# afermg/aliby

Hardware: AMD Instinct MI355X
Metric: FOV tiles/sec (whole node) (higher is better)
Workload: dtype u16 pixels, f64 feature accumulators, f32 dynamics, bfloat16 U-Net

## Files before the change

### aliby_amd/_lib.py

```python

from __future__ import annotations

import ctypes as C
import os
import threading
from pathlib import Path

import numpy as np

_HERE = Path(__file__).resolve().parent
LIB_PATH = Path(os.environ["ALIBY_HIP_LIB"]) if os.environ.get("ALIBY_HIP_LIB") else _HERE / "libaliby_hip.so"

OK, ERR_INVALID, ERR_OVERFLOW, ERR_HIP, ERR_TOO_LARGE, ERR_UNSUPPORTED = range(6)
U16, F32 = 0, 1
U8W = 4
U64, F64 = 2, 3
RED_MAX, RED_ADD, RED_DIV = 0, 1, 2


class AlibyHipError(RuntimeError):
    pass


class aliby_object(C.Structure):
    _fields_ = [
        ("tile", C.c_int32),
        ("label", C.c_int32),
        ("y0", C.c_int32),
        ("x0", C.c_int32),
        ("y1", C.c_int32),
        ("x1", C.c_int32),
        ("area", C.c_int32),
        ("pad_", C.c_int32),
    ]


class aliby_pq_column(C.Structure):
    _fields_ = [("name", C.c_char_p), ("type", C.c_int32), ("reserved", C.c_int32)]


class aliby_npy_member(C.Structure):
    _fields_ = [("name", C.c_char_p), ("descr", C.c_char_p), ("shape", C.POINTER(C.c_int64)), ("data", C.c_void_p),
                ("ndim", C.c_int32), ("itemsize", C.c_int32)]


PQ_F64, PQ_I64, PQ_U16, PQ_STR = range(4)

OBJECT_DTYPE = np.dtype(
    [("tile", "<i4"), ("label", "<i4"), ("y0", "<i4"), ("x0", "<i4"), ("y1", "<i4"), ("x1", "<i4"),
     ("area", "<i4"), ("pad_", "<i4")]
)

_vp, _i, _sz = C.c_void_p, C.c_int, C.c_size_t
_ip = C.POINTER(C.c_int32)

_SIGNATURES = {
    "aliby_abi_version": (_i, []),
    "aliby_last_error": (C.c_char_p, []),
    "aliby_ctx_create": (_i, [_i, C.POINTER(_vp)]),
    "aliby_ctx_destroy": (_i, [_vp]),
    "aliby_device_info": (_i, [_vp, C.POINTER(_i), C.POINTER(_i), C.POINTER(_sz), C.c_char_p, _i]),
    "aliby_malloc": (_i, [_vp, _sz, C.POINTER(_vp)]),
    "aliby_free": (_i, [_vp, _vp]),
    "aliby_memcpy_h2d": (_i, [_vp, _vp, _vp, _sz, _vp]),
    "aliby_memcpy_d2h": (_i, [_vp, _vp, _vp, _sz, _vp]),
    "aliby_memset": (_i, [_vp, _vp, _i, _sz, _vp]),
    "aliby_stream_sync": (_i, [_vp, _vp]),
    "aliby_crop_pad_u16": (_i, [_vp, _vp, _i, _i, _i, _i, _vp, _i, _i, _i, _vp, _vp, _vp]),
    "aliby_reduce_z": (_i, [_vp, _vp, _i, _sz, _i, _sz, _i, _vp, _i, _vp]),
    "aliby_label_max": (_i, [_vp, _vp, _i, _i, _i, _vp, _vp]),
    "aliby_object_table": (_i, [_vp, _vp, _i, _i, _i, _vp, _vp, _vp, _vp]),
    "aliby_relabel_sequential": (_i, [_vp, _vp, _i, _i, _i, _vp, _vp]),
    "aliby_select_project_u16": (_i, [_vp, _vp, _i, _i, _i, _i, _i, _i, _vp, _vp]),
    "aliby_normalize99_u16": (_i, [_vp, _vp, _i, _i, _i, C.c_double, C.c_double, _vp, _vp, _vp]),
    "aliby_make_tiles": (_i, [_vp, _vp, _i, _i, _i, _i, _i, _i, _i, _i, _i, _i, _i, _vp, _vp, _i, _vp, _vp]),
    "aliby_average_tiles": (_i, [_vp, _vp, _i, _i, _i, _i, _i, _i, _i, _i, _i, _i, _i, _vp, _vp, _vp, _vp, _vp, _vp]),
    "aliby_nn_fused_act_bf16": (_i, [_vp, _vp, _vp, _vp, _vp, _vp, _vp, _vp, _i, _i, _i, _i, _i, _i, _i, _i, _vp]),
    "aliby_nn_conv3x3_bf16": (_i, [_vp, _vp, _vp, _vp, _vp, _vp, _i, _vp, _vp, _i, _i, _i, _i, _i, _i, _i, _i, _i, _i, _i, _vp, _vp]),
    "aliby_nn_conv3x3_deep_bf16": (_i, [_vp, _vp, _vp, _vp, _vp, _vp, _i, _vp, _vp, _i, _i, _i, _i, _i, _i, _i, _vp]),
    "aliby_nn_conv3x3_deep16_bf16": (_i, [_vp, _vp, _vp, _vp, _vp, _vp, _i, _vp, _vp, _i, _i, _i, _i, _i, _i, _i, _vp]),
    "aliby_nn_pack_conv3x3_deep16_bf16": (_i, [_vp, _vp, _i, _i, _vp, _vp]),
    "aliby_nn_maxpool2_bf16": (_i, [_vp, _vp, _vp, _i, _i, _i, _i, _vp]),
    "aliby_debug_conv_deep_trace": (_i, [_vp, _vp]),
    "aliby_track_stitch": (_i, [_vp, _vp, _vp, _i, _i, _i, _vp, _vp, _vp, _vp, _vp, _vp, C.c_double, _vp, _vp, _vp]),
    "aliby_debug_conv_trace": (_i, [_vp, _vp]),
    "aliby_features_coloc_pairs": (_i, [_vp, _vp, _vp, _i, _i, _i, _i, _i, _vp, _i, _vp, _i, _i, _vp, _i, C.c_double, C.c_double, _vp, _vp, _vp]),
    "aliby_trap_gauss1d": (_i, [_vp, _vp, _vp, _i, _i, _i, _vp, _i, _i, _vp]),
    "aliby_trap_warp": (_i, [_vp, _vp, _i, _i, _vp, _i, _i, _vp, _i, C.c_double, _vp]),
    "aliby_trap_entropy": (_i, [_vp, _vp, _i, _i, _i, _vp, _vp]),
    "aliby_trap_morph": (_i, [_vp, _vp, _vp, _i, _i, _i, _i, _i, _vp]),
    "aliby_trap_label": (_i, [_vp, _vp, _i, _i, _vp, _vp]),
    "aliby_trap_region_sums": (_i, [_vp, _vp, _i, _i, _vp, _vp]),
    "aliby_trap_match_template": (_i, [_vp, _vp, _i, _i, _vp, _i, _i, _vp, _i, _i, C.c_double, C.c_double, _vp]),
    "aliby_trap_maxfilter1d": (_i, [_vp, _vp, _vp, _i, _i, _i, _i, _vp]),
    "aliby_tiff_probe": (_i, [C.c_char_p, _vp, C.c_char_p, _i]),
    "aliby_ingest_tiff_planes": (_i, [_vp, _vp, _vp, _i, _i, _i, _i, _vp, _sz, _i, _i, _vp]),
    "aliby_ingest_inflate": (_i, [_i, _vp, _sz, _vp, _sz, _vp]),
    "aliby_nn_pack_conv3x3_bf16": (_i, [_vp, _vp, _i, _i, _i, _vp, _vp]),
    "aliby_nn_pack_conv1x1_bf16": (_i, [_vp, _vp, _i, _i, _i, _vp, _vp]),
    "aliby_nn_conv3x3_proj_bf16": (_i, [_vp, _vp, _vp, _vp, _vp, _vp, _i, _vp, _i, _i, _i, _i, _i, _vp, _vp, _i, _vp]),
    "aliby_nn_conv3x3_head_bf16": (_i, [_vp, _vp, _vp, _vp, _vp, _vp, _i, _vp, _vp, _i, _i, _i, _i, _i, _i, _vp, _vp, _vp, _vp, _i, _vp, _vp]),
    "aliby_nn_conv3x3_pair_bf16": (_i, [_vp, _vp, _vp, _vp, _vp, _vp, _vp, _i, _vp, _vp, _vp, _i, _vp, _vp, _i, _i, _i, _vp, _vp, _vp, _vp, _vp,
                                        _i, _vp, _vp]),
    "aliby_nn_first_pair_bf16": (_i, [_vp, _vp, _i, _i, _i, _i, _vp, _vp, _vp, _vp, _vp, _vp, _vp, _vp, _vp, _vp]),
    "aliby_nn_conv1x1_bf16": (_i, [_vp, _vp, _vp, _vp, _vp, _i, _i, _i, _i, _i, _vp]),
    "aliby_nn_first_conv_bf16": (_i, [_vp, _vp, _i, _i, _i, _i, _vp, _vp, _vp, _vp, _vp, _vp]),
    "aliby_nn_style_bf16": (_i, [_vp, _vp, _i, _i, _i, _i, _vp, _vp, _i, _vp, _vp, _vp]),
    "aliby_nn_out_head_bf16": (_i, [_vp, _vp, _vp, _vp, _vp, _vp, _i, _i, _i, _i, _i, _vp, _vp]),
    "aliby_nn_nhwc_to_nchw_f32": (_i, [_vp, _vp, _i, _i, _i, _i, _i, _vp, _vp, _vp]),
    "aliby_nn_tiles_to_nhwc8_bf16": (_i, [_vp, _vp, _i, _i, _i, _i, _vp, _vp, _vp, _vp, _vp]),
    "aliby_masks_workspace_bytes": (_sz, [_i, _i, _i]),
    "aliby_masks_from_flows": (_i, [_vp, _vp, _vp, _i, _i, _i, _i, C.c_float, C.c_float, _i, C.c_float, _vp, _sz,
                                    _vp, _vp, _vp, _vp]),
    "aliby_features_intensity": (_i, [_vp, _vp, _vp, _i, _i, _i, _i, _i, _i, _vp, _i, _i, _i, _vp, _i, _i, _vp]),
    "aliby_features_sizeshape": (_i, [_vp, _vp, _i, _i, _i, _vp, _i, _i, _i, _i, _vp, _i, _i, _vp]),
    "aliby_features_feret": (_i, [_vp, _vp, _i, _i, _i, _vp, _i, _i, _vp, _i, _i, _vp]),
    "aliby_object_mec": (_i, [_vp, _vp, _i, _i, _i, _vp, _i, _i, _vp, _vp]),
    "aliby_features_zernike": (_i, [_vp, _vp, _vp, _i, _i, _i, _i, _i, _i, _vp, _i, _vp, _i, _vp, _i, _i, _vp]),
    "aliby_features_radial_zernikes_multi": (_i, [_vp, _vp, _vp, _i, _i, _i, _i, _i, _vp, _vp, _i, _vp, _i, _vp, _vp, _i, _vp]),
    "aliby_features_texture": (_i, [_vp, _vp, _vp, _i, _i, _i, _i, _i, _i, _vp, _i, _i, _i, _i, _i, _i, _vp, _i, _i, _vp]),
    "aliby_radial_geometry": (_i, [_vp, _vp, _i, _i, _i, _vp, _i, _i, _i, _i, _vp, _vp]),
    "aliby_features_radial_distribution": (_i, [_vp, _vp, _vp, _vp, _i, _i, _i, _i, _i, _i, _vp, _i, _i, _vp, _i, _i, _vp]),
    "aliby_features_cell_ratio": (_i, [_vp, _vp, _vp, _i, _i, _i, _i, _i, _i, _i, _vp, _i, _i, _vp, _vp]),
    "aliby_features_trap_background": (_i, [_vp, _vp, _vp, _i, _i, _i, _i, _i, _i, _vp, _vp]),
    "aliby_granularity_workspace_bytes": (_sz, [_i, _i, _i, _i, C.c_double, C.c_double]),
    "aliby_features_granularity": (_i, [_vp, _vp, _vp, _i, _i, _i, _i, _i, _i, _vp, _i, C.c_double, C.c_double, _i, _i, _i,
                                        _vp, _sz, _vp, _i, _i, _vp]),
    "aliby_radial_geometry_unscaled": (_i, [_vp, _vp, _i, _i, _i, _vp, _i, _i, _i, _i, C.c_double, _vp, _vp]),
    "aliby_features_radial_distribution_rings": (_i, [_vp, _vp, _vp, _vp, _i, _i, _i, _i, _i, _i, _vp, _i, _i, _i, _vp, _i, _i, _vp]),
    "aliby_features_cell": (_i, [_vp, _vp, _vp, _i, _i, _i, _i, _i, _i, _vp, _i, _i, _i, _i, _vp, _i, _i, _vp]),
    "aliby_features_coloc": (_i, [_vp, _vp, _vp, _i, _i, _i, _i, _i, _i, _i, _vp, _i, _i, _vp, _i, _i, _i, _i, _i,
                                  C.c_double, C.c_double, _vp, _vp, _vp]),
    "aliby_labels_apply_lut": (_i, [_vp, _vp, _i, _i, _i, _vp, _vp, _vp, _vp]),
    "aliby_features_intensity3d": (_i, [_vp, _vp, _vp, _i, _i, _i, _i, _i, _i, _vp, _vp, _i, _i, _vp]),
    "aliby_parquet_write": (_i, [C.c_char_p, _vp, _i, _vp, _i, _vp, _vp, _i]),
    "aliby_npz_write": (_i, [C.c_char_p, _vp, _i, _i]),
    "aliby_host_codecs": (_i, [C.POINTER(_i), C.POINTER(_i)]),
    "aliby_host_copy": (_i, [_vp, _vp, _sz, _i]),
    "aliby_object_ranks": (_i, [_vp, _vp, _vp, _i, _i, _i, _i, _i, _i, _vp, _i, _i, _vp, _vp, _vp]),
}

_lib = None


def exported_symbols() -> list[str]:
    return sorted(_SIGNATURES)


def load() -> C.CDLL:
    global _lib
    if _lib is not None:
        return _lib
    if not LIB_PATH.exists():
        raise AlibyHipError(
            f"{LIB_PATH} is missing: build it with `python -c 'import __graft_entry__ as g; g.build()'` "
            "(make -C aliby_amd/csrc). There is no CPU fallback for the HIP path."
        )
    try:
        import torch
    except Exception:
        pass
    lib = C.CDLL(str(LIB_PATH), mode=getattr(os, "RTLD_NOW", 2))
# ... 80 lines not shown
```

### aliby_amd/segment/fused_unet.py

```python

from __future__ import annotations

import os

import torch
import torch.nn.functional as F

from aliby_amd import _lib
from aliby_amd.extraction.engine import _ptr, _stream_ptr

CL = torch.channels_last


def _bn_affine(bn):
    s = bn.weight.float() / torch.sqrt(bn.running_var.float() + bn.eps)
    t = bn.bias.float() - bn.running_mean.float() * s
    return s.contiguous(), t.contiguous()


class _Unit:

    def __init__(self, seq, dtype, pad_in=None):
        bn, conv = seq[0], seq[-1]
        self.scale, self.shift = _bn_affine(bn)
        w = conv.weight.detach().float()
        if pad_in is not None and w.shape[1] < pad_in:
            w = F.pad(w, (0, 0, 0, 0, 0, pad_in - w.shape[1]))
            self.scale = F.pad(self.scale, (0, pad_in - self.scale.shape[0]), value=1.0)
            self.shift = F.pad(self.shift, (0, pad_in - self.shift.shape[0]))
        self.w = w.to(dtype).contiguous(memory_format=CL)
        self.w32 = w.contiguous()
        self.wpk = None
        self.bias = conv.bias.detach().float().contiguous()
        self.pad = conv.padding


class _Proj:

    def __init__(self, seq, dtype, pad_in=None):
        bn, conv = seq[0], seq[-1]
        s, t = _bn_affine(bn)
        w = conv.weight.detach().float()
        b = conv.bias.detach().float() + (w[:, :, 0, 0] @ t)
        w = w * s[None, :, None, None]
        if pad_in is not None and w.shape[1] < pad_in:
            w = F.pad(w, (0, 0, 0, 0, 0, pad_in - w.shape[1]))
        self.w = w.to(dtype).contiguous(memory_format=CL)
        self.w32 = w[:, :, 0, 0].contiguous()
        self.wpk = None
        self.wpk1 = None
        self.bias = b.contiguous()


_MFMA_SHAPES = {(32, 32, False), (32, 64, False), (64, 64, False), (64, 32, True), (64, 64, True), (64, 128, False), (64, 128, True)}
_POOL_SHAPES = {(32, 32, False), (32, 64, False), (64, 64, False), (64, 128, False)}


class FusedUNet:
    @property
    def h(self):
        return self.eng.ctx.handle

    def __init__(self, net, eng, dtype=torch.bfloat16, mfma_levels=(0, 1, 2, 3)):
        assert dtype == torch.bfloat16, "the fused kernels are bf16"
        self.eng, self.dtype = eng, dtype
        self.mfma_levels = tuple(mfma_levels)
        self.fused_head = os.environ.get("ALIBY_NET_FUSED_HEAD", "1") != "0"
        self.fused_pair = os.environ.get("ALIBY_NET_FUSED_PAIR", "1") != "0"
        self.pair_head = os.environ.get("ALIBY_NET_PAIR_HEAD", "0") != "0"
        self.fused_first = os.environ.get("ALIBY_NET_FUSED_FIRST", "1") != "0"
        self.deep_kernel = os.environ.get("ALIBY_CONV_DEEP", "1") != "0"
        self.conv_stats = {}
        self.lib = _lib.load_fast() if os.environ.get("ALIBY_FAST_LAUNCH", "1") != "0" else eng.lib
        net = net.float().eval()
        self.down = []
        for i, blk in enumerate(net.down):
            pad = 8 if i == 0 else None
            d = dict(proj=_Proj(blk.proj, dtype, pad), u=[_Unit(blk.conv[0], dtype, pad)] + [_Unit(blk.conv[k], dtype) for k in (1, 2, 3)])
            d["pb1"] = (d["proj"].bias + d["u"][1].bias).contiguous()
            d["shift1_b0"] = (d["u"][1].scale * d["u"][0].bias + d["u"][1].shift).contiguous()
            self.down.append(d)
        self.up = []
        for blk in net.up:
            d = dict(proj=_Proj(blk.proj, dtype), u=[_Unit(blk.conv0, dtype)])
            for su in (blk.conv1, blk.conv2, blk.conv3):
                u = _Unit(su.conv, dtype)
                u.full_w = su.full.weight.detach().float().t().contiguous()
                u.full_b = su.full.bias.detach().float()
                d["u"].append(u)
            d["pb1"] = (d["proj"].bias + d["u"][1].bias).contiguous()
            self.up.append(d)
        ws, bs, off = [], [], 0
        for d in self.up:
            for k in d["u"][1:]:
                ws.append(k.full_w * k.scale[None, :])
                bs.append(k.full_b * k.scale + k.shift)
                k.style_slice = (off, off + k.scale.numel())
                off += k.scale.numel()
        self.style_w = torch.cat(ws, dim=1).contiguous()
        self.style_b = torch.cat(bs).contiguous()
        self.first_w = net.down[0].conv[0][-1].weight.detach().float().to(dtype).float().contiguous()
        self.out = _Unit(net.output, dtype)
        self.out_w = self.out.w32[:, :, 0, 0].to(dtype).float().contiguous()
        self.cin = net.nbase[0]
        self.bytes_moved = 0

    def _new(self, n, c, h, w):
        return torch.empty((n, c, h, w), dtype=self.dtype, device="cuda", memory_format=CL)

    def _fused(self, A, B=None, want_sum=False, act=None, shift=None, upA=False, upB=False, relu=True, bias=None):
        n, c = A.shape[0], A.shape[1]
        H = A.shape[2] * (2 if upA else 1)
        W = A.shape[3] * (2 if upA else 1)
        S = self._new(n, c, H, W) if want_sum else None
        T = self._new(n, c, H, W) if act is not None else None
        per_sample = 0
        sh = None
        if act is not None:
            sh = shift if shift is not None else act.shift
            per_sample = self._sps(sh)
        timer = self.eng.timed("fused_pointwise")
        if timer.active:
            self.bytes_moved += 2 * (A.numel() + (B.numel() if B is not None else 0) + (n * c * H * W) * ((S is not None) + (T is not None)))
        with timer:
          _lib.check(self.lib.aliby_nn_fused_act_bf16(
            self.h, _ptr(A), _ptr(B) if B is not None else 0, _ptr(S) if S is not None else 0, _ptr(T) if T is not None else 0,
            _ptr(bias) if bias is not None else 0,
            _ptr(act.scale) if act is not None else 0, _ptr(sh) if sh is not None else 0, n, H, W, c, 1 if upA else 0,
            1 if upB else 0, 1 if relu else 0, per_sample, _stream_ptr()))
        return S, T

    @staticmethod
    def _conv(x, unit, pad=1):
        return F.conv2d(x, unit.w, None, padding=pad)

    def _proj(self, x, proj):
        n, cin, H, W = x.shape
        cout = proj.w32.shape[0]
        if cin not in (32, 64, 128, 256) or not (cout in (32, 64) or cout % 128 == 0) or proj.w32.shape[1] != cin:
            return self._conv(x, proj, pad=0)
        if proj.wpk1 is None:
            proj.wpk1 = torch.empty(cout * cin, dtype=torch.bfloat16, device="cuda")
            _lib.check(self.lib.aliby_nn_pack_conv1x1_bf16(self.h, _ptr(proj.w32), cout, cin, cin, _ptr(proj.wpk1), _stream_ptr()))
        out = self._new(n, cout, H, W)
        with self.eng.timed("conv1x1_mfma"):
            _lib.check(self.lib.aliby_nn_conv1x1_bf16(self.h, _ptr(x), _ptr(proj.wpk1), 0, _ptr(out), n, H, W, cin, cout, _stream_ptr()))
        return out

    def _unit(self, x, unit, shift=None, bias=None, res=None, res_up=False, in_up=False, pool=False):
        n, cin, cout = x.shape[0], x.shape[1], unit.w32.shape[0]
        H, W = (x.shape[2] * 2, x.shape[3] * 2) if in_up else (x.shape[2], x.shape[3])
        out = self._new(n, cout, H, W)
        pooled = self._new(n, cout, H // 2, W // 2) if pool else None
        if self.deep_kernel and cout % 128 == 0 and cin in (64, 128, 256) and W <= 56 and (H + 1) * (W + 2) >= 226 + 2 * (W + 2):
            self._launch_deep(x, unit, out, shift, bias, res, res_up, in_up)
            if pool:
                with self.eng.timed("maxpool"):
                    _lib.check(self.lib.aliby_nn_maxpool2_bf16(self.h, _ptr(out), _ptr(pooled), n, H, W, cout, _stream_ptr()))
            return (out, pooled) if pool else out
        if (cin, cout, bool(in_up)) in (_POOL_SHAPES if pool else _MFMA_SHAPES):
            self._launch_unit(x, unit, (0, cin), (0, cout), out, shift, bias, res, res_up, in_up, pooled)
            return (out, pooled) if pool else out
        ns = 128 if cout > 128 else cout
        ks = 64 if cin > 64 else cin
        assert cin % ks == 0 and cout % ns == 0 and (ks, ns, bool(in_up)) in _MFMA_SHAPES, (cin, cout, in_up)
        for n0 in range(0, cout, ns):
            cur, cur_up = res, res_up
            for k0 in range(0, cin, ks):
                last = k0 + ks == cin
                self._launch_unit(x, unit, (k0, k0 + ks), (n0, n0 + ns), out, shift, bias if last else None, cur, cur_up, in_up,
                                  pooled if last else None)
                cur, cur_up = out, False
        return (out, pooled) if pool else out

    def _pack(self, unit):
        cout, cin = unit.w32.shape[0], unit.w32.shape[1]
        if unit.wpk is None:
            unit.wpk = {}
        key = (0, cin, 0, cout)
        if key not in unit.wpk:
            pk = torch.empty(cout * cin * 9, dtype=torch.bfloat16, device="cuda")
            _lib.check(self.lib.aliby_nn_pack_conv3x3_bf16(self.h, _ptr(unit.w32), cout, cin, cin, _ptr(pk), _stream_ptr()))
            unit.wpk[key] = pk
        return unit.wpk[key]

    def _pair(self, x, ua, ub, shift_a, shift_b, bias_a, bias_b, res, pool=False, head_out=None):
        n, cin, H, W = x.shape
        sa = ua.shift if shift_a is None else shift_a
        sb = ub.shift if shift_b is None else shift_b
        out = None if head_out is not None else self._new(n, 32, H, W)
        pooled = self._new(n, 32, H // 2, W // 2) if pool else None
        group = "conv3x3_mfma_pair"
        timer = self.eng.timed(group)
        if timer.active:
            st = self.conv_stats.setdefault(group, [0, 0])
            st[0] += 2 * (x.numel() + res.numel()) + (2 * x.numel() if out is not None else 4 * head_out.numel()) + (x.numel() // 2 if pool else 0)
            st[1] += 2 * 2 * 9 * 32 * 32 * n * H * W
        hd = self.out
        with timer:
            _lib.check(self.lib.aliby_nn_conv3x3_pair_bf16(
                self.h, _ptr(x), _ptr(self._pack(ua)), _ptr(self._pack(ub)), _ptr(out) if out is not None else 0, _ptr(ua.scale), _ptr(sa),
                self._sps(sa), _ptr(bias_a), _ptr(ub.scale), _ptr(sb), self._sps(sb), _ptr(bias_b), _ptr(res), n, H, W,
                _ptr(pooled) if pooled is not None else 0,
                _ptr(hd.scale) if head_out is not None else 0, _ptr(hd.shift) if head_out is not None else 0,
                _ptr(self.out_w) if head_out is not None else 0, _ptr(hd.bias) if head_out is not None else 0,
                self.out_w.shape[0] if head_out is not None else 0, _ptr(head_out) if head_out is not None else 0, _stream_ptr()))
        return (out, pooled) if pool else out

    def _first_pair(self, tiles, d):
        n, cin, H, W = tiles.shape
        u, proj = d["u"], d["proj"]
        wpk1 = self._pack(u[1])
        if proj.wpk is None:
            proj.wpk = torch.empty(32 * 16, dtype=torch.bfloat16, device="cuda")
            _lib.check(self.lib.aliby_nn_pack_conv1x1_bf16(self.h, _ptr(proj.w32), 32, proj.w32.shape[1], 16, _ptr(proj.wpk), _stream_ptr()))
        out = self._new(n, 32, H, W)
        group = "conv3x3_mfma_first_pair"
        timer = self.eng.timed(group)
        if timer.active:
            st = self.conv_stats.setdefault(group, [0, 0])
            st[0] += 4 * tiles.numel() + 2 * out.numel()
            st[1] += 2 * (9 * cin + 9 * 32 + cin) * 32 * n * H * W
        with timer:
            _lib.check(self.lib.aliby_nn_first_pair_bf16(
                self.h, _ptr(tiles), n, cin, H, W, _ptr(u[0].scale), _ptr(u[0].shift), _ptr(self.first_w), _ptr(wpk1), _ptr(u[1].scale),
                _ptr(d["shift1_b0"]), _ptr(d["pb1"]), _ptr(proj.wpk), _ptr(out), _stream_ptr()))
        return out

    def _unit_head(self, x, unit, shift, bias, res, y):
        n, cin, H, W = x.shape
        cout = unit.w32.shape[0]
        if unit.wpk is None:
            unit.wpk = {}
        key = (0, cin, 0, cout)
        if key not in unit.wpk:
            pk = torch.empty(cout * cin * 9, dtype=torch.bfloat16, device="cuda")
            _lib.check(self.lib.aliby_nn_pack_conv3x3_bf16(self.h, _ptr(unit.w32), cout, cin, cin, _ptr(pk), _stream_ptr()))
            unit.wpk[key] = pk
        sh = unit.shift if shift is None else shift
        group = "conv3x3_mfma_head"
        timer = self.eng.timed(group)
        if timer.active:
            st = self.conv_stats.setdefault(group, [0, 0])
            st[0] += 2 * (x.numel() + res.numel()) + 4 * y.numel()
            st[1] += 2 * (9 * cin + y.shape[1]) * cout * n * H * W
        with timer:
            _lib.check(self.lib.aliby_nn_conv3x3_head_bf16(
                self.h, _ptr(x), _ptr(unit.wpk[key]), 0, _ptr(unit.scale), _ptr(sh), self._sps(sh), _ptr(bias), _ptr(res), 0, n, H, W,
                cin, cout, _ptr(self.out.scale), _ptr(self.out.shift), _ptr(self.out_w), _ptr(self.out.bias), self.out_w.shape[0], _ptr(y),
                _stream_ptr()))

    def _unit_proj(self, x, unit, shift, bias, x_in, proj):
        n, cin, H, W = x.shape
        cout = unit.w32.shape[0]
        pc_pad = 16 if cin == 32 else 32
        if unit.wpk is None:
            unit.wpk = {}
        key = (0, cin, 0, cout)
        if key not in unit.wpk:
            pk = torch.empty(cout * cin * 9, dtype=torch.bfloat16, device="cuda")
            _lib.check(self.lib.aliby_nn_pack_conv3x3_bf16(self.h, _ptr(unit.w32), cout, cin, cin, _ptr(pk), _stream_ptr()))
            unit.wpk[key] = pk
        if proj.wpk is None:
            proj.wpk = torch.empty(cout * pc_pad, dtype=torch.bfloat16, device="cuda")
            _lib.check(self.lib.aliby_nn_pack_conv1x1_bf16(self.h, _ptr(proj.w32), cout, proj.w32.shape[1], pc_pad, _ptr(proj.wpk), _stream_ptr()))
        sh = unit.shift if shift is None else shift
        out = self._new(n, cout, H, W)
        group = "conv3x3_mfma"
        timer = self.eng.timed(group)
        if timer.active:
            st = self.conv_stats.setdefault(group, [0, 0])
            st[0] += 2 * (x.numel() + out.numel() + x_in.numel())
            st[1] += 2 * (9 * cin + x_in.shape[1]) * cout * n * H * W
        with timer:
            _lib.check(self.lib.aliby_nn_conv3x3_proj_bf16(
                self.h, _ptr(x), _ptr(unit.wpk[key]), _ptr(out), _ptr(unit.scale), _ptr(sh), self._sps(sh), _ptr(bias), n, H, W, cin, cout,
                _ptr(x_in), _ptr(proj.wpk), x_in.shape[1], _stream_ptr()))
        return out

    def _launch_deep(self, x, unit, out, shift, bias, res, res_up, in_up):
        n, cin, cout = x.shape[0], x.shape[1], out.shape[1]
        H, W = out.shape[2], out.shape[3]
        sh = unit.shift if shift is None else shift
        group = "conv3x3_mfma_deep"
        timer = self.eng.timed(group)
        if timer.active:
            st = self.conv_stats.setdefault(group, [0, 0])
            st[0] += 2 * (x.numel() + out.numel() + (res.numel() if res is not None else 0))
            st[1] += 2 * 9 * cin * cout * n * H * W
        with timer:
            _lib.check(self.lib.aliby_nn_conv3x3_deep_bf16(
                self.h, _ptr(x), _ptr(self._pack(unit)), _ptr(out), _ptr(unit.scale), _ptr(sh), self._sps(sh),
                _ptr(bias) if bias is not None else 0, _ptr(res) if res is not None else 0, 1 if res_up else 0, n, H, W, cin, cout,
                1 if in_up else 0, _stream_ptr()))

    def _launch_unit(self, x, unit, kslice, nslice, out, shift, bias, res, res_up, in_up, pooled):
        n, ctot, cout_tot = x.shape[0], x.shape[1], out.shape[1]
        (k0, k1), (n0, n1) = kslice, nslice
        cin, cout = k1 - k0, n1 - n0
        H, W = out.shape[2], out.shape[3]
        assert pooled is None or (cin, cout, bool(in_up)) in _POOL_SHAPES
        if unit.wpk is None:
            unit.wpk = {}
        key = (k0, k1, n0, n1)
        if key not in unit.wpk:
            w = unit.w32[n0:n1, k0:k1].contiguous()
            pk = torch.empty(cout * cin * 9, dtype=torch.bfloat16, device="cuda")
            _lib.check(self.lib.aliby_nn_pack_conv3x3_bf16(self.h, _ptr(w), cout, w.shape[1], cin, _ptr(pk), _stream_ptr()))
            unit.wpk[key] = pk
        sh = unit.shift if shift is None else shift
        sh = sh[..., k0:k1]
        scale = unit.scale[k0:k1]
        group = "conv3x3_mfma_deep" if cout >= 128 else "conv3x3_mfma"
        timer = self.eng.timed(group)
        if timer.active:
            px_out = n * H * W
            st = self.conv_stats.setdefault(group, [0, 0])
            st[0] += 2 * (x.numel() * cin // ctot + px_out * cout + (res.numel() * cout // cout_tot if res is not None else 0)
                          + (px_out // 4 * cout if pooled is not None else 0))
            st[1] += 2 * 9 * cin * cout * px_out
        with timer:
            _lib.check(self.lib.aliby_nn_conv3x3_bf16(
                self.h, _ptr(x), _ptr(unit.wpk[key]), _ptr(out), _ptr(scale), _ptr(sh), self._sps(sh),
                _ptr(bias[n0:n1]) if bias is not None else 0, _ptr(res) if res is not None else 0, 1 if res_up else 0, n, H, W, cin, cout,
                1 if in_up else 0, ctot, k0, cout_tot, n0, _ptr(pooled) if pooled is not None else 0, _stream_ptr()))

    def _style_shift(self, unit):
        lo, hi = unit.style_slice
        return self._style_all[:, lo:hi]

    @staticmethod
    def _sps(sh):
        return 0 if sh.ndim == 1 else sh.stride(0)

    def _down_mfma(self, i, d, x_raw, x_act, x1=None):
        u = d["u"]
        if x1 is not None:
            pool = i + 1 < len(self.down) and u[3].w32.shape[0] <= 128
            if self.fused_pair and tuple(u[2].w32.shape[:2]) == (32, 32) and tuple(u[3].w32.shape[:2]) == (32, 32):
                return self._pair(x1, u[2], u[3], None, None, u[2].bias, u[3].bias, x1, pool=pool)
            c2 = self._unit(x1, u[2], bias=u[2].bias)
            return self._unit(c2, u[3], bias=u[3].bias, res=x1, pool=pool)
        fuse_proj = (u[1].w32.shape[1], u[1].w32.shape[0]) in ((32, 32), (64, 64))
        p = None if fuse_proj else self._proj(x_raw, d["proj"])
        if i == 0:
            c0 = x_act if self._first_c0 else self._conv(x_act, u[0])
            sh1 = d["shift1_b0"]
        else:
            c0 = self._unit(x_raw, u[0], bias=u[0].bias)
            sh1 = None
        if fuse_proj:
            x1 = self._unit_proj(c0, u[1], sh1, d["pb1"], x_raw, d["proj"])
        else:
            x1 = self._unit(c0, u[1], shift=sh1, bias=d["pb1"], res=p)
        pool = i + 1 < len(self.down) and u[3].w32.shape[0] <= 128
        if self.fused_pair and tuple(u[2].w32.shape[:2]) == (32, 32) and tuple(u[3].w32.shape[:2]) == (32, 32):
            return self._pair(x1, u[2], u[3], None, None, u[2].bias, u[3].bias, x1, pool=pool)
        c2 = self._unit(x1, u[2], bias=u[2].bias)
        return self._unit(c2, u[3], bias=u[3].bias, res=x1, pool=pool)

    def _up_mfma(self, d, x, skip, style, up=True, head_out=None):
        u = d["u"]
        p_low = self._proj(x, d["proj"])
        c0s = self._unit(x, u[0], bias=u[0].bias, res=skip, in_up=up)
        sh = [self._style_shift(k) for k in u[1:]]
        x1 = self._unit(c0s, u[1], shift=sh[0], bias=d["pb1"], res=p_low, res_up=up)
        pair_shapes = tuple(u[2].w32.shape[:2]) == (32, 32) and tuple(u[3].w32.shape[:2]) == (32, 32)
        if self.fused_pair and pair_shapes and (head_out is None or self.pair_head):
            return self._pair(x1, u[2], u[3], sh[1], sh[2], u[2].bias, u[3].bias, x1, head_out=head_out)
        c2 = self._unit(x1, u[2], shift=sh[1], bias=u[2].bias)
        if head_out is not None:
            self._unit_head(c2, u[3], sh[2], u[3].bias, x1, head_out)
            return None
        return self._unit(c2, u[3], shift=sh[2], bias=u[3].bias, res=x1)
# ... 105 lines not shown
```

### include/aliby_hip.h

```cpp
#ifndef ALIBY_HIP_H
#define ALIBY_HIP_H

#include <stddef.h>
#include <stdint.h>

#ifdef __cplusplus
extern "C" {
#endif

#define ALIBY_ABI_VERSION 1

enum {
  ALIBY_OK = 0,
  ALIBY_ERR_INVALID = 1,
  ALIBY_ERR_OVERFLOW = 2,
  ALIBY_ERR_HIP = 3,
  ALIBY_ERR_TOO_LARGE = 4,
  ALIBY_ERR_UNSUPPORTED = 5
};

enum { ALIBY_U16 = 0, ALIBY_F32 = 1,
       ALIBY_U64 = 2, ALIBY_F64 = 3 ,
       ALIBY_U8W = 4  };

enum { ALIBY_RED_MAX = 0, ALIBY_RED_ADD = 1, ALIBY_RED_DIV = 2 };

typedef struct aliby_ctx aliby_ctx;

typedef struct aliby_object {
  int32_t tile;
  int32_t label;
  int32_t y0, x0;
  int32_t y1, x1;
  int32_t area;
  int32_t pad_;
} aliby_object;

int aliby_abi_version(void);
const char* aliby_last_error(void);
int aliby_ctx_create(int device, aliby_ctx** out);
int aliby_ctx_destroy(aliby_ctx* ctx);
int aliby_device_info(aliby_ctx* ctx, int* cu_count, int* lds_bytes, size_t* hbm_bytes,
                      char* name, int name_len);

int aliby_malloc(aliby_ctx* ctx, size_t bytes, void** dptr);
int aliby_free(aliby_ctx* ctx, void* dptr);
int aliby_memcpy_h2d(aliby_ctx* ctx, void* dst_dev, const void* src_host, size_t bytes, void* stream);
int aliby_memcpy_d2h(aliby_ctx* ctx, void* dst_host, const void* src_dev, size_t bytes, void* stream);
int aliby_memset(aliby_ctx* ctx, void* dst_dev, int value, size_t bytes, void* stream);
int aliby_stream_sync(aliby_ctx* ctx, void* stream);

int aliby_crop_pad_u16(aliby_ctx* ctx, const uint16_t* stack, int C, int Z, int Y, int X,
                       const int32_t* rects, int F, int h, int w, uint16_t* out,
                       int32_t* nan_flags_host, void* stream);

int aliby_reduce_z(aliby_ctx* ctx, const void* in, int dtype, size_t outer, int Z, size_t inner,
                   int op, void* out, int out_dtype, void* stream);

int aliby_label_max(aliby_ctx* ctx, const uint16_t* labels, int F, int Y, int X,
                    int32_t* max_host, void* stream);
int aliby_object_table(aliby_ctx* ctx, const uint16_t* labels, int F, int Y, int X,
                       const int32_t* offsets_host, aliby_object* table_dev,
                       aliby_object* table_host, void* stream);

int aliby_relabel_sequential(aliby_ctx* ctx, uint16_t* labels, int F, int Y, int X,
                             int32_t* n_host, void* stream);

int aliby_select_project_u16(aliby_ctx* ctx, const uint16_t* pixels, int F, int C, int Z, int Y, int X,
                             int channel, uint16_t* out, void* stream);
int aliby_normalize99_u16(aliby_ctx* ctx, const uint16_t* img, int F, int Y, int X, double lower,
                          double upper, float* out, double* percentiles_dev, void* stream);
int aliby_make_tiles(aliby_ctx* ctx, const float* img, int F, int Y, int X, int ypad1, int xpad1, int Ly,
                     int Lx, int by, int bx, int ny, int nx, const int32_t* ystart_dev,
                     const int32_t* xstart_dev, int nchan, float* tiles, void* stream);
int aliby_average_tiles(aliby_ctx* ctx, const float* ytiles, int F, int Y, int X, int ypad1, int xpad1,
                        int Ly, int Lx, int by, int bx, int ny, int nx, const int32_t* ystart_dev,
                        const int32_t* xstart_dev, const float* taper_dev, float* dP, float* cellprob,
                        void* stream);

int aliby_nn_fused_act_bf16(aliby_ctx* ctx, const void* A, const void* B, void* SUM, void* ACT,
                            const float* bias, const float* scale, const float* shift, int N, int H, int W,
                            int C, int upA, int upB, int relu, int shift_per_sample, void* stream);
int aliby_nn_conv3x3_bf16(aliby_ctx* ctx, const void* in, const void* wpk, void* out, const float* scale,
                          const float* shift, int shift_per_sample, const float* bias, const void* res,
                          int res_up, int N, int H, int W, int CIN, int COUT, int in_up, int in_channels,
                          int in_channel0, int out_channels, int out_channel0, void* pool_out, void* stream);
int aliby_track_stitch(aliby_ctx* ctx, const uint16_t* prev, const uint16_t* cur, int F, int Y, int X,
                       const aliby_object* cur_table_dev, const int32_t* cur_offsets_host,
                       const aliby_object* prev_table_dev, const int32_t* prev_offsets_host,
                       const int32_t* prev_tracked_dev, const int32_t* max_label_in_host, double threshold,
                       int32_t* cur_tracked_dev, int32_t* max_label_out_host, void* stream);

int aliby_nn_conv3x3_deep_bf16(aliby_ctx* ctx, const void* in, const void* wpk, void* out, const float* scale,
                               const float* shift, int shift_per_sample, const float* bias, const void* res, int res_up,
                               int N, int H, int W, int CIN, int COUT, int in_up, void* stream);

int aliby_nn_conv3x3_deep16_bf16(aliby_ctx* ctx, const void* in, const void* wpk16, void* out, const float* scale,
                               const float* shift, int shift_per_sample, const float* bias, const void* res, int res_up,
                               int N, int H, int W, int CIN, int COUT, int in_up, void* stream);
int aliby_nn_pack_conv3x3_deep16_bf16(aliby_ctx* ctx, const float* w_oihw, int COUT, int CIN, void* wpk16, void* stream);
int aliby_debug_conv_deep_trace(aliby_ctx* ctx, void* stamps_dev);
int aliby_nn_maxpool2_bf16(aliby_ctx* ctx, const void* in, void* out, int N, int H, int W, int C, void* stream);

int aliby_debug_conv_trace(aliby_ctx* ctx, void* stamps_dev);
int aliby_nn_conv3x3_proj_bf16(aliby_ctx* ctx, const void* in, const void* wpk, void* out, const float* scale,
                               const float* shift, int shift_per_sample, const float* bias, int N, int H, int W,
                               int CIN, int COUT, const void* proj_in, const void* proj_wpk, int proj_channels,
                               void* stream);
int aliby_nn_conv3x3_head_bf16(aliby_ctx* ctx, const void* in, const void* wpk, void* out_or_null, const float* scale,
                               const float* shift, int shift_per_sample, const float* bias, const void* res, int res_up,
                               int N, int H, int W, int CIN, int COUT, const float* head_scale,
                               const float* head_shift, const float* head_w, const float* head_bias, int head_channels,
                               float* head_out, void* stream);
int aliby_nn_first_pair_bf16(aliby_ctx* ctx, const float* tiles, int N, int Cin, int H, int W, const float* scale0,
                             const float* shift0, const float* w_oihw, const void* wpk1, const float* scale1,
                             const float* shift1, const float* bias1, const void* proj_wpk, void* out, void* stream);
int aliby_nn_conv3x3_pair_bf16(aliby_ctx* ctx, const void* in, const void* wpk_a, const void* wpk_b, void* out_or_null,
                               const float* scale_a, const float* shift_a, int shift_a_per_sample, const float* bias_a,
                               const float* scale_b, const float* shift_b, int shift_b_per_sample, const float* bias_b,
                               const void* res, int N, int H, int W, void* pool_out, const float* head_scale,
                               const float* head_shift, const float* head_w, const float* head_bias, int head_channels,
                               float* head_out, void* stream);
int aliby_nn_pack_conv3x3_bf16(aliby_ctx* ctx, const float* w_oihw, int COUT, int CIN_src, int CIN, void* wpk,
                               void* stream);
int aliby_nn_pack_conv1x1_bf16(aliby_ctx* ctx, const float* w_oi, int COUT, int CIN_src, int CIN, void* wpk,
                               void* stream);
int aliby_nn_nhwc_to_nchw_f32(aliby_ctx* ctx, const void* y, int N, int H, int W, int Cpad, int Cout,
                              const float* bias, float* out, void* stream);
int aliby_nn_conv1x1_bf16(aliby_ctx* ctx, const void* in, const void* wpk, const float* bias, void* out, int N, int H, int W,
                          int CIN, int COUT, void* stream);
int aliby_nn_first_conv_bf16(aliby_ctx* ctx, const float* tiles, int N, int Cin, int H, int W, const float* scale,
                             const float* shift, const float* w_oihw, void* raw8, void* c0, void* stream);
int aliby_nn_style_bf16(aliby_ctx* ctx, const void* x, int N, int H, int W, int C, const float* wt, const float* b, int J,
                        float* style, float* shifts, void* stream);
int aliby_nn_out_head_bf16(aliby_ctx* ctx, const void* x, const float* scale, const float* shift, const float* w,
                           const float* bias, int N, int H, int W, int C, int O, float* out, void* stream);
int aliby_nn_tiles_to_nhwc8_bf16(aliby_ctx* ctx, const float* tiles, int N, int Cin, int H, int W,
                                 const float* scale, const float* shift, void* raw, void* act, void* stream);

size_t aliby_masks_workspace_bytes(int F, int Y, int X);
int aliby_masks_from_flows(aliby_ctx* ctx, const float* dP, const float* cellprob, int F, int Y, int X,
                           int niter, float cellprob_threshold, float flow_threshold, int min_size,
                           float max_size_fraction, void* workspace, size_t workspace_bytes,
                           uint16_t* labels_out, int32_t* n_labels_host, float* p_final_out, void* stream);

int aliby_features_intensity(aliby_ctx* ctx, const uint16_t* labels, const void* planes, int dtype,
                             int F, int C, int Y, int X, int channel,
                             const aliby_object* table_dev, int n_obj, int max_area,
                             int edge_measurements, double* out, int ld, int col0, void* stream);

int aliby_features_sizeshape(aliby_ctx* ctx, const uint16_t* labels, int F, int Y, int X,
                             const aliby_object* table_dev, int n_obj, int max_h, int max_w,
                             int max_area, double* out, int ld, int col0, void* stream);

int aliby_features_feret(aliby_ctx* ctx, const uint16_t* labels, int F, int Y, int X,
                         const aliby_object* table_dev, int n_obj, int max_h, double* out, int ld,
                         int col0, void* stream);

int aliby_object_mec(aliby_ctx* ctx, const uint16_t* labels, int F, int Y, int X,
                     const aliby_object* table_dev, int n_obj, int max_h, double* mec_dev, void* stream);

int aliby_features_zernike(aliby_ctx* ctx, const uint16_t* labels, const void* planes, int dtype,
                           int F, int C, int Y, int X, int channel, const aliby_object* table_dev,
                           int n_obj, const double* mec_dev, int weighted, double* out, int ld, int col0,
                           void* stream);
int aliby_features_radial_zernikes_multi(aliby_ctx* ctx, const uint16_t* labels, const void* planes, int dtype, int F, int C, int Y,
                                         int X, const int* channels, const int* col0s, int n_channels, const aliby_object* table_dev,
                                         int n_obj, const double* mec_dev, double* out, int ld, void* stream);

int aliby_features_texture(aliby_ctx* ctx, const uint16_t* labels, const void* planes, int dtype,
                           int F, int C, int Y, int X, int channel, const aliby_object* table_dev,
                           int n_obj, int max_h, int max_w, int max_area, int scale, int gray_levels,
                           double* out, int ld, int col0, void* stream);

int aliby_radial_geometry(aliby_ctx* ctx, const uint16_t* labels, int F, int Y, int X,
                          const aliby_object* table_dev, int n_obj, int max_h, int max_w, int bin_count,
                          uint8_t* binmap_dev, void* stream);
int aliby_features_radial_distribution(aliby_ctx* ctx, const uint16_t* labels, const uint8_t* binmap_dev,
// ... 95 lines not shown
```

Baseline: 599.9.

## Add persistent K-looped MFMA conv3x3 kernel for wide 128-to-64 channel layers

```diff
diff --git a/aliby_amd/_lib.py b/aliby_amd/_lib.py
--- a/aliby_amd/_lib.py
+++ b/aliby_amd/_lib.py
@@ -78,6 +78,7 @@
     "aliby_nn_fused_act_bf16": (_i, [_vp, _vp, _vp, _vp, _vp, _vp, _vp, _vp, _i, _i, _i, _i, _i, _i, _i, _i, _vp]),
     "aliby_nn_conv3x3_bf16": (_i, [_vp, _vp, _vp, _vp, _vp, _vp, _i, _vp, _vp, _i, _i, _i, _i, _i, _i, _i, _i, _i, _i, _i, _vp, _vp]),
     "aliby_nn_conv3x3_deep_bf16": (_i, [_vp, _vp, _vp, _vp, _vp, _vp, _i, _vp, _vp, _i, _i, _i, _i, _i, _i, _i, _vp]),
+    "aliby_nn_conv3x3_kloop64_bf16": (_i, [_vp, _vp, _vp, _vp, _vp, _vp, _i, _vp, _vp, _i, _i, _i, _i, _i, _i, _i, _vp]),
     "aliby_nn_conv3x3_deep16_bf16": (_i, [_vp, _vp, _vp, _vp, _vp, _vp, _i, _vp, _vp, _i, _i, _i, _i, _i, _i, _i, _vp]),
     "aliby_nn_pack_conv3x3_deep16_bf16": (_i, [_vp, _vp, _i, _i, _vp, _vp]),
     "aliby_nn_maxpool2_bf16": (_i, [_vp, _vp, _vp, _i, _i, _i, _i, _vp]),
diff --git a/aliby_amd/csrc/nn_conv_up.hip b/aliby_amd/csrc/nn_conv_up.hip
--- /dev/null
+++ b/aliby_amd/csrc/nn_conv_up.hip
@@ -0,0 +1,305 @@
+#include "common.h"
+#include <utility>
+
+typedef __bf16 bf16x8_t __attribute__((ext_vector_type(8)));
+typedef __bf16 bf16x2_t __attribute__((ext_vector_type(2)));
+typedef short s16x2_t __attribute__((ext_vector_type(2)));
+typedef float f32x16_t __attribute__((ext_vector_type(16)));
+typedef float f32x2_t __attribute__((ext_vector_type(2)));
+
+namespace {
+
+template <class F, int... I>
+__device__ __forceinline__ void uc_sfor_impl(F&& f, std::integer_sequence<int, I...>) {
+  (f(std::integral_constant<int, I>{}), ...);
+}
+template <int N, class F>
+__device__ __forceinline__ void uc_sfor(F&& f) {
+  uc_sfor_impl(static_cast<F&&>(f), std::make_integer_sequence<int, N>{});
+}
+
+__device__ __forceinline__ float uc_bf2f(unsigned h) { return __uint_as_float(h << 16); }
+__device__ __forceinline__ unsigned uc_pack2(float lo, float hi) {
+  const f32x2_t f = {lo, hi};
+  return __builtin_bit_cast(unsigned, __builtin_convertvector(f, bf16x2_t));
+}
+__device__ __forceinline__ uint4 uc_act8(uint4 v, const f32x2_t (&sc)[4], const f32x2_t (&sh)[4], unsigned keep) {
+  const unsigned w4[4] = {v.x, v.y, v.z, v.w};
+  unsigned r4[4];
+#pragma unroll
+  for (int q = 0; q < 4; ++q) {
+    const f32x2_t x = {__uint_as_float(w4[q] << 16), __uint_as_float(w4[q] & 0xffff0000u)};
+    const f32x2_t y = __builtin_elementwise_fma(sc[q], x, sh[q]);
+    s16x2_t b = __builtin_bit_cast(s16x2_t, __builtin_convertvector(y, bf16x2_t));
+    const s16x2_t zero = {0, 0};
+    b = __builtin_elementwise_max(b, zero);
+    r4[q] = __builtin_bit_cast(unsigned, b) & keep;
+  }
+  return make_uint4(r4[0], r4[1], r4[2], r4[3]);
+}
+
+struct UpArgs {
+  const uint4* in;
+  const uint4* wpk;
+  uint4* out;
+  const float* scale;
+  const float* shift;
+  const float* bias;
+  const uint4* res;
+  int shift_stride, res_up;
+  int N, H, W;
+  int LW, HP;
+  int q_begin, q_end;
+  int ntiles;
+};
+
+constexpr int UC_NB = 7;
+constexpr int UC_RUN = UC_NB * 32;
+constexpr int UC_TILE = 2 * UC_RUN;
+constexpr int UC_COUT = 64;
+constexpr int UC_KS = 32;
+constexpr int UC_WMAX = 112;
+constexpr int UC_WIN_MAX = UC_TILE + 2 * (UC_WMAX + 2) + 2;
+constexpr int UC_PLANE = UC_WIN_MAX | 1;
+constexpr int UC_POS_PER_ROUND = 256 / (UC_KS / 8);
+constexpr int UC_ITERS = (UC_WIN_MAX + UC_POS_PER_ROUND - 1) / UC_POS_PER_ROUND;
+constexpr int UC_LDS_BYTES = (UC_KS / 8) * UC_PLANE * 16 + UC_ITERS * 256 * 4;
+constexpr int UC_WDEPTH = 3;
+constexpr int UC_PDEPTH = 4;
+constexpr int UC_NW = 2 * 9;
+constexpr int UC_REQ_AT = 13;
+static_assert(UC_ITERS <= 32, "inside / later masks are 32-bit");
+
+template <int CIN, bool UP>
+__global__ __launch_bounds__(256, 2) void k_conv3x3_up(UpArgs a) {
+  constexpr int S = CIN / UC_KS, KCT = CIN / 16;
+  extern __shared__ uint4 lds[];
+  const int tid = threadIdx.x, lane = tid & 63, wave = tid >> 6;
+  const int cb = wave & 1, rr = wave >> 1;
+  const int px = lane & 31, hh = lane >> 5;
+  const int pl = tid & 3, pos0 = tid >> 2;
+  const int IH = UP ? a.H >> 1 : a.H, IW = UP ? a.W >> 1 : a.W;
+  const int LW = a.LW, HP = a.HP;
+  const int WIN = UC_TILE + 2 * LW + 2;
+  const int cs = CIN / 8;
+  int* const goff = reinterpret_cast<int*>(lds + (UC_KS / 8) * UC_PLANE) + tid;
+
+  const int xcd = blockIdx.x & 7, slot = blockIdx.x >> 3, nslots = gridDim.x >> 3;
+  const int per_xcd = (a.ntiles + 7) >> 3;
+  const int t_end = min(a.ntiles, (xcd + 1) * per_xcd);
+
+  for (int tile = xcd * per_xcd + slot; tile < t_end; tile += nslots) {
+    const int q0 = a.q_begin + tile * UC_TILE;
+    const int p_first = q0 - LW - 1;
+    unsigned inside = 0, later = 0;
+    const int n0 = max(0, ((p_first / LW) - 1) / HP);
+    {
+      const int P0 = p_first + pos0;
+      int r = P0 >= 0 ? P0 / LW : -1, c = P0 - r * LW;
+      int n = r >= 1 ? (r - 1) / HP : 0, y = r >= 1 ? (r - 1) - n * HP : r - 1;
+#pragma unroll
+      for (int it = 0; it < UC_ITERS; ++it) {
+        const bool ok = y >= 0 && y < a.H && c >= 1 && c <= a.W && n < a.N;
+        inside |= (unsigned)ok << it;
+        later |= (unsigned)(n > n0) << it;
+        const int nn = min(n, a.N - 1), yy = min(max(y, 0), a.H - 1), xx = min(max(c - 1, 0), a.W - 1);
+        goff[it * 256] = ((nn * IH + (UP ? yy >> 1 : yy)) * IW + (UP ? xx >> 1 : xx)) * cs + pl;
+        c += UC_POS_PER_ROUND;
+        while (c >= LW) {
+          c -= LW;
+          if (++y == HP) { y = 0; ++n; }
+        }
+      }
+    }
+    const int n1 = min(n0 + 1, a.N - 1);
+    uint4 v[UC_ITERS];
+    auto request = [&](int s) {
+      const uint4* inS = a.in + s * (UC_KS / 8);
+#pragma unroll
+      for (int it = 0; it < UC_ITERS; ++it) v[it] = inS[(unsigned)goff[it * 256]];
+    };
+    request(0);
+
+    const int qw = q0 + rr * UC_RUN;
+    const int c0 = cb * 32 + hh * 16;
+    constexpr int ocs = UC_COUT / 8;
+    f32x16_t acc[UC_NB];
+    {
+      float b16[16];
+#pragma unroll
+      for (int k = 0; k < 16; ++k) b16[k] = a.bias ? a.bias[c0 + k] : 0.f;
+      if (a.res) {
+        const int RH = a.H >> a.res_up, RW = a.W >> a.res_up;
+        uint4 rv[UC_NB][2];
+        {
+          const int q = qw + px;
+          int r = q / LW, c = q - r * LW;
+          int n = (r - 1) / HP, y = (r - 1) - n * HP;
+#pragma unroll
+          for (int b = 0; b < UC_NB; ++b) {
+            const int nn = min(n, a.N - 1), yy = min(y, a.H - 1), xx = min(max(c - 1, 0), a.W - 1);
+            const unsigned roff = (unsigned)(((nn * RH + (yy >> a.res_up)) * RW + (xx >> a.res_up)) * ocs + (c0 >> 3));
+            rv[b][0] = a.res[roff];
+            rv[b][1] = a.res[roff + 1];
+            c += 32;
+            while (c >= LW) {
+              c -= LW;
+              if (++y == HP) { y = 0; ++n; }
+            }
+          }
+        }
+#pragma unroll
+        for (int b = 0; b < UC_NB; ++b) {
+          const unsigned rw[8] = {rv[b][0].x, rv[b][0].y, rv[b][0].z, rv[b][0].w, rv[b][1].x, rv[b][1].y, rv[b][1].z, rv[b][1].w};
+#pragma unroll
+          for (int j = 0; j < 8; ++j) {
+            acc[b][2 * j] = b16[2 * j] + uc_bf2f(rw[j] & 0xffffu);
+            acc[b][2 * j + 1] = b16[2 * j + 1] + uc_bf2f(rw[j] >> 16);
+          }
+        }
+      } else {
+#pragma unroll
+        for (int b = 0; b < UC_NB; ++b)
+#pragma unroll
+          for (int k = 0; k < 16; ++k) acc[b][k] = b16[k];
+      }
+    }
+    const bf16x8_t* wbase = reinterpret_cast<const bf16x8_t*>(a.wpk) + (size_t)cb * 9 * KCT * 64 + lane;
+
+    for (int s = 0; s < S; ++s) {
+      const bf16x8_t* wp = wbase + (size_t)(2 * s) * 64;
+      bf16x8_t wring[UC_WDEPTH];
+      auto wfrag = [&](int i) { return wp[((i % 9) * KCT + (i / 9)) * 64]; };
+#pragma unroll
+      for (int i = 0; i < UC_WDEPTH - 1; ++i) wring[i] = wfrag(i);
+      f32x2_t sc[4], sh[4], sh1[4];
+      {
+        const int ch = s * UC_KS + pl * 8;
+        const float* sp0 = a.shift + (size_t)n0 * a.shift_stride + ch;
+        const float* sp1 = a.shift + (size_t)n1 * a.shift_stride + ch;
+#pragma unroll
+        for (int k = 0; k < 4; ++k) {
+          sc[k] = f32x2_t{a.scale[ch + 2 * k], a.scale[ch + 2 * k + 1]};
+          sh[k] = f32x2_t{sp0[2 * k], sp0[2 * k + 1]};
+          sh1[k] = f32x2_t{sp1[2 * k], sp1[2 * k + 1]};
+        }
+      }
+      __syncthreads();
+#pragma unroll
+      for (int it = 0; it < UC_ITERS; ++it) {
+        f32x2_t shs[4];
+#pragma unroll
+        for (int k = 0; k < 4; ++k) shs[k] = ((later >> it) & 1u) ? sh1[k] : sh[k];
+        const uint4 o = uc_act8(v[it], sc, shs, 0u - ((inside >> it) & 1u));
+        const int wp_ = pos0 + UC_POS_PER_ROUND * it;
+        if (wp_ < WIN) lds[pl * UC_PLANE + wp_] = o;
+      }
+      __syncthreads();
+
+      const bf16x8_t* L = reinterpret_cast<const bf16x8_t*>(lds) + hh * UC_PLANE + rr * UC_RUN + px;
+      const int row_off[3] = {0, LW, 2 * LW};
+      constexpr int NF = UC_NW * UC_NB;
+      bf16x8_t pring[UC_PDEPTH];
+      auto pfrag = [&](int f) {
+        const int i = f / UC_NB, b = f % UC_NB, kc = i / 9, tap = i % 9;
+        return L[2 * kc * UC_PLANE + b * 32 + row_off[tap / 3] + tap % 3];
+      };
+#pragma unroll
+      for (int f = 0; f < UC_PDEPTH - 1; ++f) pring[f] = pfrag(f);
+      uc_sfor<UC_NW>([&](auto ic) {
+        constexpr int i = decltype(ic)::value;
+        if constexpr (i == UC_REQ_AT) {
+          if (s + 1 < S) request(s + 1);
+          __builtin_amdgcn_sched_barrier(0);
+        }
+        if constexpr (i + UC_WDEPTH - 1 < UC_NW) wring[(i + UC_WDEPTH - 1) % UC_WDEPTH] = wfrag(i + UC_WDEPTH - 1);
+        uc_sfor<UC_NB>([&](auto bc) {
+          constexpr int b = decltype(bc)::value, f = i * UC_NB + b;
+          if constexpr (f + UC_PDEPTH - 1 < NF) pring[(f + UC_PDEPTH - 1) % UC_PDEPTH] = pfrag(f + UC_PDEPTH - 1);
+          acc[b] = __builtin_amdgcn_mfma_f32_32x32x16_bf16(wring[i % UC_WDEPTH], pring[f % UC_PDEPTH], acc[b], 0, 0, 0);
+        });
+        __builtin_amdgcn_sched_barrier(0);
+      });
+    }
+
+    __builtin_amdgcn_sched_barrier(0);
+    {
+      const int q = qw + px;
+      int r = q / LW, c = q - r * LW;
+      int n = (r - 1) / HP, y = (r - 1) - n * HP;
+#pragma unroll
+      for (int b = 0; b < UC_NB; ++b) {
+        const int x = c - 1;
+        const bool ok = qw + b * 32 + px < a.q_end && y < a.H && x >= 0 && x < a.W && n < a.N;
+        if (ok) {
+          uint4* op = a.out + (unsigned)(((n * a.H + y) * a.W + x) * ocs + (c0 >> 3));
+          op[0] = make_uint4(uc_pack2(acc[b][0], acc[b][1]), uc_pack2(acc[b][2], acc[b][3]), uc_pack2(acc[b][4], acc[b][5]),
+                             uc_pack2(acc[b][6], acc[b][7]));
+          op[1] = make_uint4(uc_pack2(acc[b][8], acc[b][9]), uc_pack2(acc[b][10], acc[b][11]), uc_pack2(acc[b][12], acc[b][13]),
+                             uc_pack2(acc[b][14], acc[b][15]));
+        }
+        c += 32;
+        while (c >= LW) {
+          c -= LW;
+          if (++y == HP) { y = 0; ++n; }
+        }
+      }
+    }
+  }
+}
+
+template <int CIN, bool UP>
+int launch_up(UpArgs& a, hipStream_t stream) {
+  static bool attr_done = false;
+  if (!attr_done) {
+    HIP_TRY(hipFuncSetAttribute(reinterpret_cast<const void*>(&k_conv3x3_up<CIN, UP>), hipFuncAttributeMaxDynamicSharedMemorySize,
+                                UC_LDS_BYTES));
+    attr_done = true;
+  }
+  const int per_xcd = (a.ntiles + 7) / 8;
+  const int nslots = per_xcd < 64 ? per_xcd : 64;
+  hipLaunchKernelGGL((k_conv3x3_up<CIN, UP>), dim3(8 * nslots), dim3(256), UC_LDS_BYTES, stream, a);
+  KERNEL_CHECK();
+  return ALIBY_OK;
+}
+
+}
+
+extern "C" int aliby_nn_conv3x3_kloop64_bf16(aliby_ctx* ctx, const void* in, const void* wpk, void* out, const float* scale,
+                                             const float* shift, int shift_per_sample, const float* bias, const void* res, int res_up,
+                                             int N, int H, int W, int CIN, int COUT, int in_up, void* stream_) {
+  hipStream_t stream = static_cast<hipStream_t>(stream_);
+  ARG_CHECK(ctx && in && wpk && out && scale && shift, "conv3x3_kloop64: null argument");
+  ARG_CHECK(N > 0 && H > 0 && W > 0, "conv3x3_kloop64: empty shape");
+  ARG_CHECK(!in_up || ((H & 1) == 0 && (W & 1) == 0), "conv3x3_kloop64: upsampled input needs even H, W");
+  ARG_CHECK(!res || !res_up || ((H & 1) == 0 && (W & 1) == 0), "conv3x3_kloop64: upsampled residual needs even H, W");
+  if (!(CIN == 64 || CIN == 128) || COUT != UC_COUT || W > UC_WMAX) {
+    aliby_set_error("conv3x3_kloop64: unsupported (CIN=%d, COUT=%d, W=%d): CIN in {64,128}, COUT = 64, W <= %d", CIN, COUT, W, UC_WMAX);
+    return ALIBY_ERR_UNSUPPORTED;
+  }
+  if (shift_per_sample != 0 && (long long)(H + 1) * (W + 2) < UC_TILE + 2 * (W + 2) + 2) {
+    aliby_set_error("conv3x3_kloop64: images of %dx%d are smaller than one tile window (a window may span two images at most)", H, W);
+    return ALIBY_ERR_UNSUPPORTED;
+  }
+  UpArgs a;
+  a.in = static_cast<const uint4*>(in);
+  a.wpk = static_cast<const uint4*>(wpk);
+  a.out = static_cast<uint4*>(out);
+  a.scale = scale;
+  a.shift = shift;
+  a.bias = bias;
+  a.res = static_cast<const uint4*>(res);
+  a.shift_stride = shift_per_sample == 1 ? CIN : shift_per_sample;
+  a.res_up = res_up ? 1 : 0;
+  a.N = N; a.H = H; a.W = W;
+  a.LW = W + 2;
+  a.HP = H + 1;
+  const long long rows = (long long)N * a.HP + 1;
+  ARG_CHECK(rows * a.LW < (1ll << 30), "conv3x3_kloop64: batch too large for 32-bit flat positions");
+  ARG_CHECK((long long)N * H * W * (CIN > COUT ? CIN : COUT) / 8 < (1ll << 31), "conv3x3_kloop64: tensor too large for 32-bit offsets");
+  a.q_begin = a.LW;
+  a.q_end = (int)((rows - 1) * a.LW);
+  a.ntiles = (a.q_end - a.q_begin + UC_TILE - 1) / UC_TILE;
+  if (CIN == 64) return in_up ? launch_up<64, true>(a, stream) : launch_up<64, false>(a, stream);
+  return in_up ? launch_up<128, true>(a, stream) : launch_up<128, false>(a, stream);
+}
diff --git a/aliby_amd/segment/fused_unet.py b/aliby_amd/segment/fused_unet.py
--- a/aliby_amd/segment/fused_unet.py
+++ b/aliby_amd/segment/fused_unet.py
@@ -70,6 +70,7 @@
         self.pair_head = os.environ.get("ALIBY_NET_PAIR_HEAD", "0") != "0"
         self.fused_first = os.environ.get("ALIBY_NET_FUSED_FIRST", "1") != "0"
         self.deep_kernel = os.environ.get("ALIBY_CONV_DEEP", "1") != "0"
+        self.kloop64 = os.environ.get("ALIBY_CONV_KLOOP64", "1") != "0"
         self.conv_stats = {}
         self.lib = _lib.load_fast() if os.environ.get("ALIBY_FAST_LAUNCH", "1") != "0" else eng.lib
         net = net.float().eval()
@@ -158,6 +159,9 @@
                 with self.eng.timed("maxpool"):
                     _lib.check(self.lib.aliby_nn_maxpool2_bf16(self.h, _ptr(out), _ptr(pooled), n, H, W, cout, _stream_ptr()))
             return (out, pooled) if pool else out
+        if self.deep_kernel and self.kloop64 and not pool and cout == 64 and cin == 128 and 56 < W <= 112:
+            self._launch_deep(x, unit, out, shift, bias, res, res_up, in_up, kloop64=True)
+            return out
         if (cin, cout, bool(in_up)) in (_POOL_SHAPES if pool else _MFMA_SHAPES):
             self._launch_unit(x, unit, (0, cin), (0, cout), out, shift, bias, res, res_up, in_up, pooled)
             return (out, pooled) if pool else out
@@ -278,7 +282,7 @@
                 _ptr(x_in), _ptr(proj.wpk), x_in.shape[1], _stream_ptr()))
         return out
 
-    def _launch_deep(self, x, unit, out, shift, bias, res, res_up, in_up):
+    def _launch_deep(self, x, unit, out, shift, bias, res, res_up, in_up, kloop64=False):
         n, cin, cout = x.shape[0], x.shape[1], out.shape[1]
         H, W = out.shape[2], out.shape[3]
         sh = unit.shift if shift is None else shift
@@ -289,7 +293,7 @@
             st[0] += 2 * (x.numel() + out.numel() + (res.numel() if res is not None else 0))
             st[1] += 2 * 9 * cin * cout * n * H * W
         with timer:
-            _lib.check(self.lib.aliby_nn_conv3x3_deep_bf16(
+            _lib.check((self.lib.aliby_nn_conv3x3_kloop64_bf16 if kloop64 else self.lib.aliby_nn_conv3x3_deep_bf16)(
                 self.h, _ptr(x), _ptr(self._pack(unit)), _ptr(out), _ptr(unit.scale), _ptr(sh), self._sps(sh),
                 _ptr(bias) if bias is not None else 0, _ptr(res) if res is not None else 0, 1 if res_up else 0, n, H, W, cin, cout,
                 1 if in_up else 0, _stream_ptr()))
diff --git a/include/aliby_hip.h b/include/aliby_hip.h
--- a/include/aliby_hip.h
+++ b/include/aliby_hip.h
@@ -94,6 +94,10 @@
 int aliby_nn_conv3x3_deep_bf16(aliby_ctx* ctx, const void* in, const void* wpk, void* out, const float* scale,
                                const float* shift, int shift_per_sample, const float* bias, const void* res, int res_up,
                                int N, int H, int W, int CIN, int COUT, int in_up, void* stream);
+
+int aliby_nn_conv3x3_kloop64_bf16(aliby_ctx* ctx, const void* in, const void* wpk, void* out, const float* scale,
+                                  const float* shift, int shift_per_sample, const float* bias, const void* res, int res_up,
+                                  int N, int H, int W, int CIN, int COUT, int in_up, void* stream);
 
 int aliby_nn_conv3x3_deep16_bf16(aliby_ctx* ctx, const void* in, const void* wpk16, void* out, const float* scale,
                                const float* shift, int shift_per_sample, const float* bias, const void* res, int res_up,
```

Measured after the change: 607.7 (median of 6 runs). 1.3% higher.
